# Complexity-ML/complexity-tokenizer

Measured on AMD Instinct MI355X. Metric: MB/s raw UTF-8 encoded (encode_batch), 50k ByteLevel BPE, 1/2/4/8 MI355X, higher is better.
Workload: dtype u8

## Files before the change

complexity-tokenizer_amd/csrc/ctok_internal.h:

```cpp
#pragma once
#include <hip/hip_runtime.h>

#include <cstdint>

namespace ctok_dev {

constexpr uint64_t kEmpty = ~0ull;
constexpr uint32_t kIdBits = 21;
constexpr uint64_t kKeyMask = (1ull << 42) - 1;
constexpr uint32_t kNoRank = 0x3FFFFFu;
constexpr uint32_t kMaxId = (1u << kIdBits) - 2;
constexpr uint32_t kPanicVal = kNoRank - 1;

constexpr uint32_t kErrPanic = 1u;

constexpr int kTileWords = 62;
constexpr int kTile = kTileWords * 64;
constexpr int kTileSlots = 4096;
constexpr int kSegWaves = 4;
constexpr int kSegUnroll = 4;
constexpr int kShortMax = 32;
constexpr int kMedMax = 64;
constexpr uint32_t kCap0 = kTile, kCap1 = (kTile + 8) / 9, kCap2 = (kTile + 16) / 17, kCap3 = (kTile + 32) / 33;
constexpr uint32_t kCap0Lean = 1040;
constexpr int kNumClasses = 4;
constexpr int kNumCounters = 32;
constexpr int kC3Shards = 64;
constexpr int kCounterWords = kNumCounters + kC3Shards;
__host__ __device__ constexpr int ctr_stat(int c) { return c < 3 ? 6 + 2 * c : 16; }
__host__ __device__ constexpr int ctr_chunk(int c) { return c < 3 ? 13 + c : 18; }
constexpr int kCtrLong = 0;
constexpr int kCtrErr = 2;
constexpr int kCtrNfcDocs = 3;
constexpr int kCtrDropped = 4;
constexpr int kCtrPieces = 5;
constexpr int kCtrNfcFlag = 12;
constexpr int kCtrAnyMid = 19;
constexpr int kCtrAnyC3 = 20;
constexpr int kCtrEmptyDocs = 21;
constexpr int kCtrC3Count = 22;
constexpr int kCtrC3Take = 23;
constexpr uint32_t kC3SparseDefault = 65536;
constexpr uint32_t kWgRecWords = 4 * 1024 * 4;
constexpr int kMidPackedDefault = 2;
constexpr int kOverlapDefault = 1;
constexpr int kCtrSink = 31;
constexpr int kCtrOverflow = 25;
constexpr int kCtrLongIds = 26;
constexpr int kCtrLwWords = 27;
constexpr int kCtrRounds = 29;
constexpr int kLhBuckets = 65;
constexpr int kLhHist = 0, kLhScan = 80, kLhFill = 160, kLhTake = 240, kLhWords = 320;
__host__ __device__ inline uint32_t long_bucket(uint32_t n) { return n > 4096 ? 0u : 64u - (n - 1) / 64; }
__host__ __device__ inline uint32_t list_entry(uint32_t sl, uint32_t o, uint32_t n) { return sl | (o << 12) | (n << 24); }
__host__ __device__ inline uint32_t ent_len(uint32_t e) { return (e >> 24) & 127u; }
__host__ __device__ inline uint32_t ent_ord(uint32_t e) { return (e >> 12) & 0xFFFu; }
__host__ __device__ inline uint32_t long_ord(uint64_t e) { return (uint32_t)(e >> 32) & 0xFFFu; }
__host__ __device__ inline uint32_t long_len(uint64_t e) { return (uint32_t)(e >> 44) & 0x7FFFFu; }

constexpr uint32_t kRecLong = 0x40000000u, kRecLongMask = kRecLong - 1u;
constexpr uint32_t kRecMerged32 = 0xFFFFFFFFu, kRecMerged16 = 0xFFFFu;
__host__ __device__ inline uint32_t region_base(uint2 r, int cls) {
  return cls <= 0 ? 0u : cls == 1 ? (r.x & 0xFFFFu) : cls == 2 ? (r.x >> 16) : r.y;
}
__host__ __device__ inline uint32_t rec_short(uint32_t count, uint32_t sl) { return count | (sl << 16); }

__host__ __device__ inline uint32_t mul24(uint32_t a, uint32_t b) {
#if defined(__HIP_DEVICE_COMPILE__)
  return __umul24(a, b);
#else
  return (a & 0xFFFFFFu) * (b & 0xFFFFFFu);
#endif
}

__host__ __device__ inline uint32_t mhash(uint32_t a, uint32_t b) {
  uint32_t h = mul24(a, 0x9E3779u) + mul24(b ^ 0x5A5A5Au, 0x85EBCBu);
  h ^= h >> 15;
  h = mul24(h, 0xC2B2AFu) ^ (h >> 9);
  return h ^ (h >> 16);
}
__host__ __device__ inline uint32_t mhash2(uint32_t h1) {
  uint32_t h = mul24(h1 ^ (h1 >> 24), 0x27D4EBu) + (h1 >> 11);
  h ^= h >> 13;
  h = mul24(h, 0x165667u) ^ (h >> 8);
  return h ^ (h >> 16);
}

constexpr uint32_t kHotBuckets = 4096;
constexpr uint32_t kBloomBits = 1u << 18;
constexpr uint32_t kHotU64 = 2 * kHotBuckets;
constexpr uint32_t kBloomWords = kBloomBits / 32;
constexpr uint32_t kLdsImageBytes = kHotU64 * 8 + kBloomWords * 4;
constexpr uint32_t kSortCap = 8192;

__host__ __device__ inline uint32_t key16(uint32_t a, uint32_t b) { return (a << 16) | b; }
__host__ __device__ inline uint32_t hash16_h(uint32_t a, uint32_t b) {
  const uint32_t h = mul24(a, 0x9E3779u) + mul24(b, 0x85EBCBu);
  return h ^ (h >> 13);
}
__host__ __device__ inline uint32_t hash16_g(uint32_t a, uint32_t b) {
  return mul24(b, 0xC2B2AFu) + mul24(a ^ 0x5A5Au, 0x27D4EBu);
}

__host__ __device__ inline uint32_t piece_hash(uint32_t lo, uint32_t hi, uint32_t len) {
  uint32_t h = mul24(lo, 0x9E3779u) + mul24((lo >> 24) | (hi << 8), 0x85EBCBu) + mul24((hi >> 16) | (len << 16), 0xC2B2AFu);
  h ^= h >> 15;
  h = mul24(h, 0x27D4EBu) ^ (h >> 9);
  return h ^ (h >> 16);
}

__host__ __device__ __forceinline__ int cp_range_class(uint32_t cp) {
  if (cp - 0x4E00u < 0x5200u) return 1;
  if (cp - 0xAC00u < 0x2BA4u) return 1;
  if (cp - 0x3041u < 0x56u) return 1;
  if (cp - 0x30A1u < 0x5Au) return 1;
  if (cp - 0x1F300u < 0x350u) return 3;
  return -1;
}

struct Tables {
  const uint64_t* merge_tab;
  uint32_t merge_mask;
  const uint4* lds_image;
  const uint32_t* pair0;
  const uint4* lds16_image;
  const uint64_t* merge16;
  uint32_t merge16_mask;
  const uint4* piece_tab;
  uint32_t piece_mask;
  const uint32_t* rank_newid;
  uint32_t n_ranks;
  const int32_t* byte2id;
  const uint8_t* cls_s1;
  const uint8_t* cls_s2;
  const uint8_t* nfc_s1;
  const uint16_t* nfc_s2;
  const uint8_t* cls_bmp;
  uint32_t cp_fast;
  const uint32_t* decomp_cp;
  const uint16_t* decomp_off;
  const uint32_t* decomp_data;
  uint32_t n_decomp;
  const uint64_t* comp_key;
  const uint32_t* comp_val;
  uint32_t n_comp;
  const uint8_t* bytemap_alnum;
  const uint8_t* at_bytes;
  const uint32_t* at_off;
  const uint32_t* at_id;
  const uint8_t* at_flags;
  uint32_t n_at;
  uint32_t proper;
  const uint32_t* eager;
  uint32_t window;
  const uint32_t* wmeta;
  uint32_t compact;
  uint32_t narrow;
  uint32_t short_packed;
  uint32_t mid_packed;
  uint32_t dbg;
  uint32_t all_bytes;
};

__host__ __device__ inline bool mid_folded(const Tables& t, uint32_t long_pieces) {
  return t.mid_packed == 2 && t.short_packed && t.n_at == 0 && long_pieces == 0;
}

struct Work {
  const uint8_t* text;
  uint32_t n_bytes;
  const uint64_t* doc_off;
  uint32_t n_docs;
  uint32_t* tfirst;
  uint32_t* pbits;
  uint32_t n_words;
  uint32_t n_tiles;
  uint32_t n_cus;
  uint32_t nfc_watch;
  uint32_t* nfc_bits;
  uint32_t mid_wide;
  uint32_t short_wgs;
  uint32_t chunk_sort;
  uint32_t keep_first;
  uint16_t* wpref;
  uint32_t* tile_np;
  uint32_t* tile_tok;
  uint32_t* tile_doc;
  uint32_t* tcls;
  uint32_t* list0;
  uint32_t k0;
  uint32_t* list1;
  uint32_t* list2;
  uint32_t* list3;
  void* prec;
  uint32_t rec16;
  uint32_t* mrec;
  uint32_t* pdoc;
  uint32_t* tcnt;
  uint32_t* long_cnt;
  uint32_t* long_ord;
  uint32_t* long_hist;
  uint32_t* scratch;
  uint32_t* lids;
  uint32_t* long_pos;
  uint32_t* lw_pos;
  uint32_t* rend;
  uint2* tregion;
  uint32_t long_cap, mid_cap;
  uint32_t unit;
  uint64_t* long_list;
  uint64_t* mid_list;
  uint32_t* counters;
  uint32_t* lw;
  uint32_t* scan_tmp;
  uint64_t scan_tmp_cap;
  uint64_t* stamps;
  uint32_t c3_max;
  uint32_t* c3q;
  uint32_t* c3pre;
  uint64_t* host_res;
  uint64_t* wgrec;
  uint32_t* report;
  uint32_t seq;
};

struct Lx {
  hipEvent_t start = nullptr, stop = nullptr;
};

constexpr uint32_t kDecLenMask = 0xFFFFFFu, kDecNonAscii = 1u << 30, kDecSpecial = 1u << 31;
constexpr uint32_t kDecOptSkipSpecial = 1u, kDecOptCleanup = 2u;
constexpr int kDecChunk = 4096;
constexpr int kDecTile = 4096;

struct DecTables {
  const uint2* ent;
  uint32_t n_ent;
  const uint8_t* bytes;
};

struct DecWork {
  const uint32_t* ids;
  uint32_t n_ids;
  const uint64_t* tok_off;
  uint32_t n_docs;
  uint32_t opts;
  uint32_t n_chunks;
  uint32_t* chunk_off;
  uint8_t* raw;
  uint32_t n_raw;
  uint64_t* raw_off;
  uint32_t* delbits;
  uint32_t n_tiles;
  uint32_t* tile_cnt;
  uint32_t* counters;
};

hipError_t launch_dec_len(const DecWork& w, const DecTables& t, uint32_t* tmp, uint64_t tmp_cap, hipStream_t s);
hipError_t launch_dec_gather(const DecWork& w, const DecTables& t, uint8_t* dst, uint64_t* dst_off, hipStream_t s);
hipError_t launch_dec_prepare(const DecWork& w, hipStream_t s);
hipError_t launch_dec_count(const DecWork& w, uint32_t* tmp, uint64_t tmp_cap, hipStream_t s);
hipError_t launch_dec_write(const DecWork& w, uint8_t* out, uint64_t* out_off, hipStream_t s);

constexpr uint32_t kPadItemA = 0xFFFFFFFFu;
constexpr int kPadMaxItems = 16;

struct PadWork {
  const uint32_t* ids;
  const uint64_t* tok_off;
  uint32_t n_rows;
  uint32_t pairs;
  uint32_t use_tpl;
  uint32_t n_items;
  uint32_t items[kPadMaxItems];
  uint32_t mark;
  const uint32_t* special_ids;
  uint32_t n_special;
  uint32_t truncate;
  uint64_t max_len;
  uint64_t target;
  uint32_t pad_left;
  uint32_t pad_id;
  uint64_t width;
  uint32_t* out_ids;
  uint32_t* out_attn;
  uint32_t* out_type;
  uint32_t* out_special;
  uint64_t* row_len;
  uint32_t* counters;
};
hipError_t launch_pad_len(const PadWork& w, hipStream_t s);
hipError_t launch_pad_rows(const PadWork& w, hipStream_t s);

struct WinWork {
  PadWork p;
  uint64_t stride;
  const uint32_t* tokenless;
  uint32_t n_tokenless;
  uint64_t ids_bound;
  uint64_t* row_win;
  uint64_t n_windows;
  uint64_t* win_len;
  uint32_t* win_row;
  uint64_t* win_start;
};
hipError_t launch_win_len(const WinWork& w, hipStream_t s);
hipError_t launch_win_rows(const WinWork& w, hipStream_t s);

void upload_done();
hipError_t launch_docstart(const Work& w, hipStream_t s, bool zero_counters, Lx x = {}, Lx x2 = {});
uint64_t nfc_bits_words(uint64_t n_bytes);
hipError_t scan_tiles(const Work& w, hipStream_t s, bool count, Lx x = {});
hipError_t launch_nfc_check(const uint8_t* text, uint64_t n_bytes, const uint64_t* doc_off, uint32_t n_docs,
                            const Tables& t, uint32_t* doc_flag, uint32_t* counter, hipStream_t s);
hipError_t launch_norm(const uint8_t* text, const uint64_t* doc_off, uint32_t n_docs, const uint32_t* doc_flag,
                       int add_prefix, int nfc, const Tables& t, uint32_t* cp_scratch, uint32_t* ncp,
                       uint64_t* new_len_then_off, uint8_t* out_text, int phase, hipStream_t s);
hipError_t launch_segment(const Work& w, const Tables& t, hipStream_t s, Lx x = {});
hipError_t launch_bpe_class(const Work& w, const Tables& t, int cls, hipStream_t s, Lx x = {});
hipError_t launch_report(const Work& w, hipStream_t s);
hipError_t launch_c3_sparse(const Work& w, const Tables& t, uint32_t n_pieces, hipStream_t s, Lx x = {});
hipError_t launch_long_prep(const Work& w, const Tables& t, hipStream_t s, uint32_t n_long, uint32_t* lwn,
                            uint32_t* tmp, uint64_t tmp_cap);
hipError_t launch_bpe_long(const Work& w, const Tables& t, hipStream_t s, uint32_t n_long, bool any_c3, bool any_gmem);
hipError_t launch_emit(const Work& w, uint32_t* ids, uint64_t ids_cap, uint64_t* tok_off, hipStream_t s,
                       bool count_pieces, bool empty_docs = true, Lx first = {}, Lx last = {});
hipError_t scan_u32(const uint32_t* in, uint32_t* out, uint64_t n_max, const uint32_t* n_dev,
                    uint32_t* tmp, uint64_t tmp_cap, hipStream_t s);
hipError_t scan_u64(uint64_t* inout, uint64_t n, uint64_t* tmp, uint64_t tmp_cap, hipStream_t s);
uint64_t scan_tmp_elems(uint64_t n_max);
uint64_t tile_scan_tmp_elems(uint64_t n_tiles);
hipError_t shift_u64(uint64_t* p, uint64_t n, uint64_t delta, hipStream_t s);
hipError_t launch_flag_docs(const uint64_t* off, uint64_t n_docs, const uint32_t* nfc_bits, uint32_t* flag, hipStream_t s);
hipError_t launch_flag_len(const uint64_t* off, const uint32_t* flag, uint64_t n_docs, uint64_t* len, hipStream_t s);
hipError_t launch_gather_flagged(const uint8_t* text, const uint64_t* off, const uint32_t* rank, const uint64_t* sub_pos,
                                 uint64_t n_docs, uint8_t* sub_text, uint64_t* sub_off, hipStream_t s);
hipError_t launch_splice(const uint32_t* rank, const uint64_t* main_off, const uint32_t* main_ids, const uint64_t* sub_off,
                         const uint32_t* sub_ids, uint64_t n_docs, uint32_t* ids, uint64_t ids_cap, uint64_t* out_off,
                         uint64_t* tmp, uint64_t tmp_cap, hipStream_t s);
hipError_t wire16(const uint32_t* ids, uint64_t n_ids, uint16_t* ids16, const uint64_t* toff, uint64_t n_off,
                  uint32_t* toff32, hipStream_t s);

}
```

complexity-tokenizer_amd/csrc/segment.hip:

```cpp
#include "dev_common.h"
#include "seg_lane.h"

namespace ctok_dev {


__global__ __launch_bounds__(256) void k_tilefirst(const uint64_t* __restrict__ off, uint32_t n_docs, uint32_t n_tiles,
                                                   uint32_t* __restrict__ tfirst, uint32_t* __restrict__ counters) {
  const uint32_t d = blockIdx.x * blockDim.x + threadIdx.x;
  bool empty = false;
  if (d <= n_docs && n_tiles) {
    const uint64_t y = off[d];
    empty = d < n_docs && y == off[d + 1];
    const uint64_t t_lo = d ? (off[d - 1] + 64) / kTile + 1 : 0ull;
    const uint64_t t_hi = min((y + 64) / kTile, (uint64_t)n_tiles - 1);
    for (uint64_t t = t_lo; t <= t_hi && t < t_lo + 64; t++) tfirst[t] = d;
  } else if (d < n_docs) {
    empty = off[d] == off[d + 1];
  }
  const uint64_t me = __ballot(empty);
  if (me && (threadIdx.x & 63) == (uint32_t)__ffsll((unsigned long long)me) - 1)
    atomicAdd(&counters[kCtrEmptyDocs], (uint32_t)__popcll(me));
}

__device__ uint32_t tile_first_search(const uint64_t* off, uint32_t n_docs, uint32_t tile) {
  const uint64_t key = tile ? (uint64_t)tile * kTile - 64 : 0ull;
  uint32_t lo = 0, hi = n_docs;
  while (lo < hi) {
    const uint32_t mid = lo + (hi - lo) / 2;
    if (__builtin_amdgcn_readfirstlane((uint32_t)(off[mid] < key))) lo = mid + 1;
    else hi = mid;
  }
  return lo;
}

__device__ __forceinline__ void clear_words(uint32_t* __restrict__ p, uint64_t n) {
  const uint64_t n4 = n / 4;
  uint4* p4 = reinterpret_cast<uint4*>(p);
  for (uint64_t i = (uint64_t)blockIdx.x * 256 + threadIdx.x; i < n4; i += (uint64_t)gridDim.x * 256)
    p4[i] = make_uint4(0u, 0u, 0u, 0u);
  if (blockIdx.x == 0 && threadIdx.x < n - 4 * n4) p[4 * n4 + threadIdx.x] = 0u;
}

__global__ __launch_bounds__(256) void k_clear(uint32_t* __restrict__ bits, uint64_t n, uint32_t* __restrict__ counters,
                                               uint32_t* __restrict__ tfirst, uint32_t n_tiles) {
  if (bits) clear_words(bits, n);
  for (uint32_t i = blockIdx.x * 256 + threadIdx.x; i < n_tiles; i += gridDim.x * 256) tfirst[i] = ~0u;
  if (blockIdx.x == 0 && counters && threadIdx.x < (uint32_t)kCounterWords) counters[threadIdx.x] = 0u;
}

uint64_t nfc_bits_words(uint64_t n_bytes) { return (n_bytes + 2047) / 2048 + 8; }

hipError_t launch_docstart(const Work& w, hipStream_t s, bool zero_counters, Lx x, Lx x2) {
  const bool nfc = w.nfc_watch == 2;
  const uint64_t n = nfc ? nfc_bits_words(w.n_bytes) : 0;
  const uint64_t work = std::max<uint64_t>(n / 4, w.n_tiles);
  launch_lx(x, k_clear, (unsigned)std::min<uint64_t>((work + 255) / 256 + 1, 8ull * w.n_cus), 256, 0, s,
            nfc ? w.nfc_bits : nullptr, n, zero_counters ? w.counters : nullptr, w.tfirst, w.n_tiles);
  if (w.n_tiles) launch_lx(x2, k_tilefirst, (w.n_docs + 1 + 255) / 256, 256, 0, s, w.doc_off, w.n_docs, w.n_tiles, w.tfirst, w.counters);
  else if (w.n_docs)
    k_tilefirst<<<(w.n_docs + 255) / 256, 256, 0, s>>>(w.doc_off, w.n_docs, 0, w.tfirst, w.counters);
  return hipGetLastError();
}


__device__ __forceinline__ uint32_t piece_probe(const Tables& t, uint4 e, uint32_t h, uint32_t lo, uint32_t hi,
                                                uint32_t n) {
  while (e.z != 0) {
    if (e.x == lo && e.y == hi && e.z == n) return e.w;
    h = (h + 1) & t.piece_mask;
    e = t.piece_tab[h];
  }
  return kNone;
}

__device__ __forceinline__ uint32_t select_bit(uint64_t x, uint32_t k) {
  uint32_t pos = 0;
  uint32_t lo = (uint32_t)x, hi = (uint32_t)(x >> 32);
  uint32_t c = __popc(lo);
  uint32_t v = lo;
  if (k >= c) { k -= c; v = hi; pos = 32; }
#pragma unroll
  for (int wdt = 16; wdt >= 1; wdt >>= 1) {
    const uint32_t m = (1u << wdt) - 1u;
    c = __popc(v & m);
    if (k >= c) { k -= c; v >>= wdt; pos += wdt; }
  }
  return pos;
}




#ifdef CTOK_SEG_STAMPS
#define SEG_STAMP(k)                                                                              \
  do {                                                                                            \
    __builtin_amdgcn_sched_barrier(0);                                                            \
    unsigned long long t_;                                                                        \
    asm volatile("s_memtime %0\n\ts_waitcnt lgkmcnt(0)" : "=s"(t_)::"memory");                     \
    __builtin_amdgcn_sched_barrier(0);                                                            \
    if (w.stamps && lane == 0) w.stamps[(size_t)tile * 8 + (k)] = t_;                            \
  } while (0)
#else
#define SEG_STAMP(k) do { } while (0)
#endif
template <bool R16>
__global__ __launch_bounds__(64 * kSegWaves) __attribute__((amdgpu_waves_per_eu(7))) void k_segment(Work w, Tables t) {
  __shared__ uint16_t s_pos_all[kSegWaves][64 * kSegUnroll + 8];
  __shared__ __attribute__((aligned(16))) uint32_t s_text_all[kSegWaves][(kTileWords + 2) * 16 + 8];
  __shared__ uint64_t s_D_all[kSegWaves][64];
  constexpr uint32_t kSegLongCap = 32;
  __shared__ uint64_t s_long_all[kSegWaves][kSegLongCap];
  const uint32_t lane = threadIdx.x & 63;
  const uint32_t wid = uni(threadIdx.x >> 6);
  const uint32_t tile = uni(blockIdx.x * kSegWaves + wid);
  if (tile >= w.n_tiles) return;
  uint16_t* s_pos = s_pos_all[wid];
  SEG_STAMP(0);
  const uint32_t B = w.n_bytes;
  const uint32_t t0 = tile * kTile;
  const int64_t g = (int64_t)tile * kTileWords - 1 + lane;
  const bool first = lane == 0, last = lane == 63;

  uint32_t x[16];
  uint64_t D, valid;
  {
    const int64_t x0 = g * 64;
    if (x0 >= 0 && x0 + 64 <= (int64_t)B) {
      const uint4* p = reinterpret_cast<const uint4*>(w.text + x0);
#pragma unroll
      for (int k = 0; k < 4; k++) {
        const uint4 v = p[k];
        x[4 * k] = v.x; x[4 * k + 1] = v.y; x[4 * k + 2] = v.z; x[4 * k + 3] = v.w;
      }
      valid = ~0ull;
    } else {
#pragma unroll
      for (int k = 0; k < 16; k++) x[k] = 0;
      valid = 0;
      if (x0 >= 0 && x0 < (int64_t)B) {
        const uint32_t n = B - (uint32_t)x0;
        valid = (1ull << n) - 1;
        for (uint32_t i = 0; i < n; i++) x[i >> 2] |= (uint32_t)w.text[x0 + i] << (8 * (i & 3));
      }
    }
  }
  uint32_t dfirst = uni(w.tfirst[tile]);
  if (dfirst == ~0u) dfirst = tile_first_search(w.doc_off, w.n_docs, tile);
  uint64_t xs0 = ~0ull, ys0 = ~0ull;
  if (dfirst + lane < w.n_docs) {
    xs0 = w.doc_off[dfirst + lane];
    ys0 = w.doc_off[dfirst + lane + 1];
  }
  seg::Masks m = seg::ascii_masks(x);
  {
    uint64_t* s_D = s_D_all[wid];
    s_D[lane] = 0;
    __builtin_amdgcn_fence(__ATOMIC_RELEASE, "wavefront");
    __builtin_amdgcn_wave_barrier();
    const uint64_t base = (uint64_t)t0 - 64;
    const uint64_t lim = (uint64_t)t0 + 4032;
    auto mark = [&](uint64_t xs, uint64_t ys) {
      const bool in = xs < lim;
      if (in && xs != ys) {
        const uint64_t r = xs - base;
        atomicOr((unsigned long long*)&s_D[r >> 6], 1ull << (r & 63));
      }
      return in;
    };
    if (__ballot(mark(xs0, ys0)) == ~0ull) {
      for (uint32_t d = dfirst + 64;; d += 64) {
        const uint32_t i = d + lane;
        uint64_t xs = ~0ull, ys = ~0ull;
        if (i < w.n_docs) {
          xs = w.doc_off[i];
          ys = w.doc_off[i + 1];
        }
        if (__ballot(mark(xs, ys)) != ~0ull) break;
      }
    }
    __builtin_amdgcn_fence(__ATOMIC_RELEASE, "wavefront");
    __builtin_amdgcn_wave_barrier();
    __builtin_amdgcn_fence(__ATOMIC_ACQUIRE, "wavefront");
    const int64_t x0 = g * 64;
    if (x0 < 0) D = 0;
    else if (x0 >= (int64_t)B) D = ~0ull;
    else D = s_D[lane] | ~valid;
  }
  s_D_all[wid][lane] = D;
  uint32_t* s_all = s_text_all[wid] + 4;
  uint32_t* s_text = s_all + 16;
  if (first && (x[0] & 0xC0u) == 0x80u && g * 64 >= 4)
    s_all[-1] = *reinterpret_cast<const uint32_t*>(w.text + g * 64 - 4);
#pragma unroll
  for (int k = 0; k < 4; k++)
    *reinterpret_cast<uint4*>(s_all + lane * 16 + 4 * k) = make_uint4(x[4 * k], x[4 * k + 1], x[4 * k + 2], x[4 * k + 3]);
  if (last) {
    const int64_t xe = g * 64 + 64;
    uint32_t v = 0;
    if (xe + 4 <= (int64_t)B) {
      v = *reinterpret_cast<const uint32_t*>(w.text + xe);
    } else {
      for (int64_t i = xe; i < (int64_t)B && i < xe + 4; i++) v |= (uint32_t)w.text[i] << (8 * (uint32_t)(i - xe));
    }
    s_all[64 * 16] = v;
  }
  __builtin_amdgcn_fence(__ATOMIC_RELEASE, "wavefront");
  __builtin_amdgcn_wave_barrier();
  __builtin_amdgcn_fence(__ATOMIC_ACQUIRE, "wavefront");
  SEG_STAMP(1);
  if (m.NA) {
    constexpr int kSegCp = 4;
    bool nfc_bad = false;
    auto set_class = [&](int cl, uint64_t bits) {
      if (cl == 0) m.W |= bits & m.NA;
      else if (cl == 1) m.L |= bits & m.NA;
      else if (cl == 2) m.N |= bits & m.NA;
    };
    uint64_t cont = 0;
#pragma unroll
    for (int k = 0; k < 16; k += 2) {
      const uint32_t c0 = x[k] & ~(x[k] << 1) & seg::kHi, c1 = x[k + 1] & ~(x[k + 1] << 1) & seg::kHi;
      cont |= (uint64_t)seg::pack8(c0, c1) << (4 * k);
    }
    cont &= m.NA;
    const uint64_t lead_cont = cont & ~(cont + 1);
    if (lead_cont) {
      const uint32_t pw = s_all[lane * 16 - 1];
      const int32_t back = ((pw >> 24) & 0xC0u) != 0x80u ? 1 : ((pw >> 16) & 0xC0u) != 0x80u ? 2 : 3;
      const int32_t a = (int32_t)lane * 64 - back;
      const uint32_t v = __builtin_amdgcn_alignbyte(s_all[(a >> 2) + 1], s_all[a >> 2], (uint32_t)a & 3u);
      const uint32_t b0 = v & 255u, b1 = (v >> 8) & 0x3Fu, b2 = (v >> 16) & 0x3Fu, b3 = (v >> 24) & 0x3Fu;
      const int l = u8len((uint8_t)b0);
      const uint32_t c = l == 2 ? ((b0 & 0x1Fu) << 6) | b1
                       : l == 3 ? ((b0 & 0x0Fu) << 12) | (b1 << 6) | b2
                       : l == 4 ? ((b0 & 0x07u) << 18) | (b1 << 12) | (b2 << 6) | b3 : b0;
      const int rc = t.cp_fast ? cp_range_class(c) : -1;
      const int cw = rc >= 0 ? rc : (cls_of(c, t) | (nfc16(t, c) != 0 ? 4 : 0));
      nfc_bad |= (cw & 4) != 0;
      set_class(cw & 3, lead_cont);
    }
    uint64_t leads = m.NA & ~cont;
    while (leads) {
      uint32_t pos[kSegCp], cp[kSegCp], len[kSegCp];
#pragma unroll
      for (int k = 0; k < kSegCp; k++) {
        pos[k] = leads ? (uint32_t)__builtin_ctzll(leads) : 64u;
        leads &= leads ? leads - 1 : 0ull;
      }
#pragma unroll
      for (int k = 0; k < kSegCp; k++) {
        const uint32_t a = lane * 64 + min(pos[k], 63u);
        const uint32_t v = __builtin_amdgcn_alignbyte(s_all[(a >> 2) + 1], s_all[a >> 2], a & 3);
        const uint32_t b0 = v & 255u, b1 = (v >> 8) & 0x3Fu, b2 = (v >> 16) & 0x3Fu, b3 = (v >> 24) & 0x3Fu;
        const int l = u8len((uint8_t)b0);
        len[k] = (uint32_t)l;
        cp[k] = l == 2 ? ((b0 & 0x1Fu) << 6) | b1
              : l == 3 ? ((b0 & 0x0Fu) << 12) | (b1 << 6) | b2
              : l == 4 ? ((b0 & 0x07u) << 18) | (b1 << 12) | (b2 << 6) | b3 : b0;
      }
      int rc[kSegCp];
      uint32_t s1[kSegCp];
#pragma unroll
      for (int k = 0; k < kSegCp; k++) {
        rc[k] = t.cp_fast ? cp_range_class(cp[k]) : -1;
        const bool in = pos[k] < 64 && cp[k] < 0x110000 && rc[k] < 0;
        s1[k] = in && cp[k] < 0x10000 ? (uint32_t)t.cls_bmp[cp[k] >> 1] : 0u;
      }
#pragma unroll
      for (int k = 0; k < kSegCp; k++) {
        if (pos[k] >= 64) continue;
        const uint32_t c = cp[k];
        int cl = 3;
        bool nf = false;
        if (rc[k] >= 0) {
          cl = rc[k];
        } else if (c < 0x80) {
          cl = cls_ascii(c);
        } else if (c < 0x10000) {
          const uint32_t v = s1[k] >> ((c & 1u) * 4);
          cl = (int)(v & 3u);
          nf = (v & 4u) != 0;
        } else if (c < 0x110000) {
          cl = cls_of(c, t);
          nf = nfc16(t, c) != 0;
        }
        nfc_bad |= nf;
        const uint32_t p = pos[k];
        const uint64_t bits = (len[k] >= 64 - p ? ~0ull : ((1ull << len[k]) - 1)) << p;
        set_class(cl, bits);
      }
    }
    if (nfc_bad && w.nfc_watch) {
      atomicOr(&w.counters[kCtrNfcFlag], 1u);
      if (w.nfc_watch == 2 && g >= 0) atomicOr(&w.nfc_bits[g >> 5], 1u << (g & 31));
    }
  }
  SEG_STAMP(2);
  uint64_t pQ = shfl_up64(m.Q);
  if (first) pQ = 0;
  seg::Letters lt{0, 0, 0, 0, 0};
  if (m.Q | (pQ >> 62)) lt = seg::letter_masks(x, m.NA);

  uint64_t st;
  {
    uint64_t pW = shfl_up64(m.W), pL = shfl_up64(m.L), pN = shfl_up64(m.N);
    if (first) pW = pL = pN = 0;
    uint64_t nW = shfl_down64(m.W), nL = shfl_down64(m.L), nD = shfl_down64(D);
    seg::Letters nl{shfl_down64(lt.T1), shfl_down64(lt.R), shfl_down64(lt.Le), shfl_down64(lt.V), shfl_down64(lt.LL)};
    if (last) {
      nW = nL = nD = 0;
      nl = seg::Letters{0, 0, 0, 0, 0};
    }
    const uint64_t A = seg::attached(m, D, pW, nW, nD);
    uint64_t pA = shfl_up64(A);
    if (first) pA = 0;
    uint64_t C1, C2;
    seg::contractions(m, lt, D, A, pA, ~(pW | pL | pN), nL, nD, nl, C1, C2);
    uint64_t pC1 = shfl_up64(C1), pC2 = shfl_up64(C2);
    if (first) pC1 = pC2 = 0;
    st = seg::starts(m, D, pW, pL, pN, A, pA, C1, C2, pC1, pC2) & valid;
    if (last) st &= (1ull << 62) - 1;
    if (!first && !last) {
      const uint64_t gw = (uint64_t)g * 2;
      if (gw < w.n_words) w.pbits[gw] = (uint32_t)st;
      if (gw + 1 < w.n_words) w.pbits[gw + 1] = (uint32_t)(st >> 32);
    }
  }
  uint32_t nd = (!first && !last) ? (uint32_t)__popcll(D & valid) : 0u;
  const uint32_t c = (!first && !last) ? (uint32_t)__popcll(st) : 0u;
  const uint32_t inc = wave_incl_scan(c);
  if (!first && !last) w.wpref[(size_t)tile * 64 + lane - 1] = (uint16_t)(inc - c);
  const uint32_t np = lane63(inc);
  const uint32_t tile_end =
      uni((uint32_t)__shfl((int)(st ? (uint32_t)(kTileWords * 64 + __builtin_ctzll(st))
                                    : ((uint64_t)B <= (uint64_t)t0 + kTile + 62 ? (uint32_t)(B - t0) : 0xFFFFu)),
                           63, 64));
  const uint64_t stw = (!first && !last) ? st : 0ull;
  const uint32_t prew = inc - c;
  uint32_t wcur = 1;

  SEG_STAMP(3);
  const bool generic = t.n_at != 0;
  using RecT = typename std::conditional<R16, uint16_t, uint32_t>::type;
  RecT* prec = (RecT*)w.prec + (size_t)tile * kTileSlots;
  uint32_t* pdoc = w.pdoc + (size_t)tile * (kTileSlots / 32);
  uint32_t hits = 0;
  uint32_t nm = 0;
  uint32_t n0 = 0, n1 = 0, n2 = 0, n3 = 0;
  uint32_t nlong = 0;
  uint32_t by0 = 0, by1 = 0, by2 = 0;
  constexpr int U = kSegUnroll;
  constexpr uint32_t W = 64 * U;
  for (uint32_t j0 = 0; j0 < np; j0 += W) {
    for (uint32_t wb = wcur;; wb += 32) {
      const uint32_t wl = wb + (lane >> 1), src = min(wl, 63u);
      const uint32_t lo32 = (uint32_t)__shfl((int)(uint32_t)stw, (int)src, 64);
      const uint32_t hi32 = (uint32_t)__shfl((int)(uint32_t)(stw >> 32), (int)src, 64);
      const uint32_t pw = (uint32_t)__shfl((int)prew, (int)src, 64);
      const bool hi = (lane & 1) != 0;
      uint32_t bits = wl <= (uint32_t)kTileWords ? (hi ? hi32 : lo32) : 0u;
      uint32_t k = pw + (hi ? (uint32_t)__popc(lo32) : 0u);
      if (k > j0 + W || k + (uint32_t)__popc(bits) <= j0) bits = 0;
      const uint32_t pos0 = (wl - 1) * 64 + (hi ? 32u : 0u);
      while (bits) {
        const uint32_t b = (uint32_t)__builtin_ctz(bits);
        if (k >= j0 && k <= j0 + W) s_pos[k - j0] = (uint16_t)(pos0 + b);
        bits &= bits - 1u;
        k++;
      }
      const uint32_t wn = wb + 32;
      if (wn > (uint32_t)kTileWords || uni(__builtin_amdgcn_readlane(prew, wn)) > j0 + W) break;
    }
    {
      const uint64_t inw = __ballot(lane >= wcur && lane <= (uint32_t)kTileWords && prew <= j0 + W);
      if (inw) wcur = 63u - (uint32_t)__builtin_clzll(inw);
    }

    if (lane == 0 && np <= j0 + W) s_pos[np - j0] = (uint16_t)tile_end;
    __builtin_amdgcn_fence(__ATOMIC_RELEASE, "wavefront");
    __builtin_amdgcn_wave_barrier();
    __builtin_amdgcn_fence(__ATOMIC_ACQUIRE, "wavefront");
    uint32_t sl[U], n[U], cls[U], plo[U], phi[U], h[U], doc[U];
#pragma unroll
    for (int u = 0; u < U; u++) {
      const uint32_t j = j0 + 64 * u + lane;
      sl[u] = 0;
      n[u] = 0;
      doc[u] = 0;
      cls[u] = 4;
      if (j < np) {
        sl[u] = s_pos[64 * u + lane];
        doc[u] = (uint32_t)(s_D_all[wid][(sl[u] >> 6) + 1] >> (sl[u] & 63)) & 1u;
        const uint32_t el = s_pos[64 * u + lane + 1];
        if (el == 0xFFFFu || el - sl[u] > (generic ? (uint32_t)kShortMax : (uint32_t)kMedMax)) {
          cls[u] = 3;
        } else {
          n[u] = el - sl[u];
          cls[u] = generic ? 0 : n[u] > 32 ? 6 : n[u] > 16 ? 2 : n[u] > 8 ? 1 : 5;
        }
      }
      const uint32_t a = sl[u] >> 2, sh = sl[u] & 3;
      const uint32_t d0 = s_text[a], d1 = s_text[a + 1], d2 = s_text[a + 2];
      const uint32_t w0 = __builtin_amdgcn_alignbyte(d1, d0, sh), w1 = __builtin_amdgcn_alignbyte(d2, d1, sh);
      const uint32_t nn = n[u];
      plo[u] = nn >= 4 ? w0 : w0 & ((1u << (8 * nn)) - 1u);
      phi[u] = nn >= 8 ? w1 : nn <= 4 ? 0u : w1 & ((1u << (8 * (nn - 4))) - 1u);
      h[u] = cls[u] == 5 ? piece_hash(plo[u], phi[u], nn) & t.piece_mask : t.piece_mask + 1;
    }
    uint32_t hitv[U];
#define CTOK_PROBE_LOAD(u) const uint4 e##u = t.piece_tab[h[u]];
#define CTOK_PROBE_USE(u) hitv[u] = piece_probe(t, e##u, h[u], plo[u], phi[u], n[u]);
    static_assert(U == 4 || U == 8, "kSegUnroll: 4 or 8");
    CTOK_PROBE_LOAD(0) CTOK_PROBE_LOAD(1) CTOK_PROBE_LOAD(2) CTOK_PROBE_LOAD(3)
    if constexpr (U == 8) {
      CTOK_PROBE_LOAD(4) CTOK_PROBE_LOAD(5) CTOK_PROBE_LOAD(6) CTOK_PROBE_LOAD(7)
      CTOK_PROBE_USE(4) CTOK_PROBE_USE(5) CTOK_PROBE_USE(6) CTOK_PROBE_USE(7)
    }
    CTOK_PROBE_USE(0) CTOK_PROBE_USE(1) CTOK_PROBE_USE(2) CTOK_PROBE_USE(3)
#undef CTOK_PROBE_LOAD
#undef CTOK_PROBE_USE
#pragma unroll
    for (int u = 0; u < U; u++) {
      const uint32_t j = j0 + 64 * u + lane;
      uint32_t rec = kRecMerged32;
      if (cls[u] == 5) {
        const bool hit = hitv[u] != kNone;
        rec = hit ? hitv[u] : kRecMerged32;
        hits += hit ? 1u : 0u;
        cls[u] = hit ? 4u : 0u;
      }
      if (j < np) {
        prec[j] = (RecT)rec;
      }
      const uint64_t dm = __ballot(j < np && doc[u]);
      if (lane == 0 && j0 + 64 * u < np)
        *reinterpret_cast<uint2*>(pdoc + ((j0 + 64 * u) >> 5)) = make_uint2((uint32_t)dm, (uint32_t)(dm >> 32));
    }
    {
      uint32_t tot0 = n0;
#pragma unroll
      for (int u = 0; u < U; u++) tot0 += (uint32_t)__popcll(__ballot(cls[u] == 0));
      if (tot0 > w.k0) {
        uint32_t c = n0;
#pragma unroll
        for (int u = 0; u < U; u++) {
          const uint64_t m = __ballot(cls[u] == 0);
          if (cls[u] == 0 && c + __popcll(m & lanemask_lt()) >= w.k0) cls[u] = 3;
          c += (uint32_t)__popcll(m);
        }
      }
    }
#pragma unroll
    for (int u = 0; u < U; u++) {
      const uint64_t below = lanemask_lt();
      const uint64_t mm = __ballot(cls[u] != 4);
      const uint32_t ord = nm + (uint32_t)__popcll(mm & below);
      nm += (uint32_t)__popcll(mm);
      const uint32_t e = list_entry(sl[u], ord, n[u]);
      {
        const uint64_t m0 = __ballot(cls[u] == 0);
        const uint64_t m1 = __ballot(cls[u] == 1), m2 = __ballot(cls[u] == 2);
        const uint64_t m3 = __ballot(cls[u] == 6);
        if (cls[u] == 0) w.list0[(size_t)tile * w.k0 + n0 + __popcll(m0 & below)] = e;
        if (cls[u] == 1) w.list1[(size_t)tile * kCap1 + n1 + __popcll(m1 & below)] = e;
        if (cls[u] == 2) w.list2[(size_t)tile * kCap2 + n2 + __popcll(m2 & below)] = e;
        if (cls[u] == 6) w.list3[(size_t)tile * kCap3 + n3 + __popcll(m3 & below)] = e;
        by0 += cls[u] == 0 ? n[u] : 0u;
        by1 += cls[u] == 1 ? n[u] : 0u;
        by2 += cls[u] == 2 ? n[u] : 0u;
        n0 += __popcll(m0);
        n1 += __popcll(m1);
        n2 += __popcll(m2);
        n3 += __popcll(m3);
      }
      const uint64_t lm = __ballot(cls[u] == 3);
      if (lm && nlong + (uint32_t)__popcll(lm) <= kSegLongCap) {
        if (cls[u] == 3) {
          const uint32_t el = s_pos[64 * u + lane + 1];
          const uint32_t ln = el == 0xFFFFu ? 0u : min(el - sl[u], 0x7FFFFu);
          s_long_all[wid][nlong + __popcll(lm & lanemask_lt())] =
              (uint64_t)(t0 + sl[u]) | ((uint64_t)ord << 32) | ((uint64_t)ln << 44);
        }
        nlong += (uint32_t)__popcll(lm);
      } else if (lm) {
        const uint32_t leader = __ffsll((unsigned long long)lm) - 1;
        uint32_t b = 0;
        if (lane == leader) b = atomicAdd(&w.counters[kCtrLong], (uint32_t)__popcll(lm));
        b = __builtin_amdgcn_readlane(b, leader);
        const uint32_t li = b + __popcll(lm & lanemask_lt());
        if (cls[u] == 3 && li < w.long_cap)
        {
          const uint32_t el = s_pos[64 * u + lane + 1];
          const uint32_t ln = el == 0xFFFFu ? 0u : min(el - sl[u], 0x7FFFFu);
          w.long_list[li] = (uint64_t)(t0 + sl[u]) | ((uint64_t)ord << 32) | ((uint64_t)ln << 44);
        }
        if (lane == leader && b + __popcll(lm) > w.long_cap) atomicOr(&w.counters[kCtrOverflow], 1u);
      }
    }
    __builtin_amdgcn_fence(__ATOMIC_RELEASE, "wavefront");
    __builtin_amdgcn_wave_barrier();
    __builtin_amdgcn_fence(__ATOMIC_ACQUIRE, "wavefront");
  }
  if (nlong) {
    uint32_t b = 0;
    if (lane == 0) b = atomicAdd(&w.counters[kCtrLong], nlong);
    b = __builtin_amdgcn_readfirstlane(b);
    __builtin_amdgcn_fence(__ATOMIC_RELEASE, "wavefront");
    __builtin_amdgcn_wave_barrier();
    __builtin_amdgcn_fence(__ATOMIC_ACQUIRE, "wavefront");
    if (lane < nlong && b + lane < w.long_cap) w.long_list[b + lane] = s_long_all[wid][lane];
    if (lane == 0 && b + nlong > w.long_cap) atomicOr(&w.counters[kCtrOverflow], 1u);
  }
  SEG_STAMP(4);
  hits = wave_sum_full_u32(hits);
  by0 = wave_sum_full_u32(by0);
  by1 = wave_sum_full_u32(by1);
  by2 = wave_sum_full_u32(by2);
  nd = wave_sum_full_u32(nd);
  if (lane == 0) {
    w.tile_tok[tile] = hits;
    w.tile_doc[tile] = nd;
    w.tile_np[tile] = np;
    w.tregion[tile] = make_uint2(by0 | ((by0 + by1) << 16), by0 + by1 + by2);
  }
  if (lane < kNumClasses)
    w.rend[(size_t)lane * w.n_tiles + tile] = lane == 0 ? 0u : lane == 1 ? by0 : lane == 2 ? by0 + by1 : by0 + by1 + by2;
  if (lane < kNumClasses)
    w.tcls[(size_t)lane * w.n_tiles + tile] = lane == 0 ? n0 : lane == 1 ? n1 : lane == 2 ? n2 : n3;
  if (lane == 0 && n2) w.counters[kCtrAnyMid] = 1;
  if (lane == 0 && n3) w.counters[kCtrAnyC3] = 1;
  if (n3 && w.c3_max) {
    const uint32_t sh = tile & (kC3Shards - 1), cap = w.c3_max / kC3Shards;
    uint32_t b = 0;
    if (lane == 0) b = atomicAdd(&w.counters[kNumCounters + sh], n3);
    b = __builtin_amdgcn_readfirstlane(b);
    for (uint32_t j = lane; j < n3; j += 64)
      if (b + j < cap) w.c3q[(size_t)sh * cap + b + j] = (tile << 7) | j;
  }
  SEG_STAMP(5);
#ifdef CTOK_SEG_STAMPS
  if (w.stamps && lane == 0) w.stamps[(size_t)tile * 8 + 6] = np;
#endif
}

hipError_t launch_segment(const Work& w, const Tables& t, hipStream_t s, Lx x) {
  const uint32_t grid = (w.n_tiles + kSegWaves - 1) / kSegWaves;
  if (w.n_tiles && w.rec16) launch_lx(x, k_segment<true>, grid, 64 * kSegWaves, 0, s, w, t);
  else if (w.n_tiles) launch_lx(x, k_segment<false>, grid, 64 * kSegWaves, 0, s, w, t);
  return hipGetLastError();
}

}
```

Before: 176,500.

## Compact non-hit pieces into LDS buffer before emitting class lists

```diff
diff --git a/complexity-tokenizer_amd/csrc/ctok_internal.h b/complexity-tokenizer_amd/csrc/ctok_internal.h
--- a/complexity-tokenizer_amd/csrc/ctok_internal.h
+++ b/complexity-tokenizer_amd/csrc/ctok_internal.h
@@ -19,6 +19,10 @@
 constexpr int kTileSlots = 4096;
 constexpr int kSegWaves = 4;
 constexpr int kSegUnroll = 4;
+constexpr uint32_t kSegListBuf = 64 * kSegUnroll;
+__host__ __device__ inline uint32_t seg_mark(uint32_t sl, uint32_t cls) { return sl | (cls << 12); }
+__host__ __device__ inline uint32_t seg_mark_start(uint32_t m) { return m & 0xFFFu; }
+__host__ __device__ inline uint32_t seg_mark_class(uint32_t m) { return m >> 12; }
 constexpr int kShortMax = 32;
 constexpr int kMedMax = 64;
 constexpr uint32_t kCap0 = kTile, kCap1 = (kTile + 8) / 9, kCap2 = (kTile + 16) / 17, kCap3 = (kTile + 32) / 33;
diff --git a/complexity-tokenizer_amd/csrc/segment.hip b/complexity-tokenizer_amd/csrc/segment.hip
--- a/complexity-tokenizer_amd/csrc/segment.hip
+++ b/complexity-tokenizer_amd/csrc/segment.hip
@@ -71,6 +71,12 @@
     e = t.piece_tab[h];
   }
   return kNone;
+}
+
+__device__ __forceinline__ void seg_wave_sync() {
+  __builtin_amdgcn_fence(__ATOMIC_RELEASE, "wavefront");
+  __builtin_amdgcn_wave_barrier();
+  __builtin_amdgcn_fence(__ATOMIC_ACQUIRE, "wavefront");
 }
 
 __device__ __forceinline__ uint32_t select_bit(uint64_t x, uint32_t k) {
@@ -110,6 +116,7 @@
   __shared__ uint64_t s_D_all[kSegWaves][64];
   constexpr uint32_t kSegLongCap = 32;
   __shared__ uint64_t s_long_all[kSegWaves][kSegLongCap];
+  __shared__ uint8_t s_buf_all[kSegWaves][kSegListBuf];
   const uint32_t lane = threadIdx.x & 63;
   const uint32_t wid = uni(threadIdx.x >> 6);
   const uint32_t tile = uni(blockIdx.x * kSegWaves + wid);
@@ -178,9 +185,7 @@
         if (__ballot(mark(xs, ys)) != ~0ull) break;
       }
     }
-    __builtin_amdgcn_fence(__ATOMIC_RELEASE, "wavefront");
-    __builtin_amdgcn_wave_barrier();
-    __builtin_amdgcn_fence(__ATOMIC_ACQUIRE, "wavefront");
+    seg_wave_sync();
     const int64_t x0 = g * 64;
     if (x0 < 0) D = 0;
     else if (x0 >= (int64_t)B) D = ~0ull;
@@ -204,9 +209,7 @@
     }
     s_all[64 * 16] = v;
   }
-  __builtin_amdgcn_fence(__ATOMIC_RELEASE, "wavefront");
-  __builtin_amdgcn_wave_barrier();
-  __builtin_amdgcn_fence(__ATOMIC_ACQUIRE, "wavefront");
+  seg_wave_sync();
   SEG_STAMP(1);
   if (m.NA) {
     constexpr int kSegCp = 4;
@@ -326,7 +329,7 @@
       if (gw + 1 < w.n_words) w.pbits[gw + 1] = (uint32_t)(st >> 32);
     }
   }
-  uint32_t nd = (!first && !last) ? (uint32_t)__popcll(D & valid) : 0u;
+  const uint32_t nd = uni(wave_sum_full_u32((!first && !last) ? (uint32_t)__popcll(D & valid) : 0u));
   const uint32_t c = (!first && !last) ? (uint32_t)__popcll(st) : 0u;
   const uint32_t inc = wave_incl_scan(c);
   if (!first && !last) w.wpref[(size_t)tile * 64 + lane - 1] = (uint16_t)(inc - c);
@@ -344,13 +347,67 @@
   using RecT = typename std::conditional<R16, uint16_t, uint32_t>::type;
   RecT* prec = (RecT*)w.prec + (size_t)tile * kTileSlots;
   uint32_t* pdoc = w.pdoc + (size_t)tile * (kTileSlots / 32);
-  uint32_t hits = 0;
   uint32_t nm = 0;
   uint32_t n0 = 0, n1 = 0, n2 = 0, n3 = 0;
   uint32_t nlong = 0;
-  uint32_t by0 = 0, by1 = 0, by2 = 0;
+  uint32_t by01 = 0, by2h = 0;
   constexpr int U = kSegUnroll;
   constexpr uint32_t W = 64 * U;
+  static_assert(U == 4, "kSegUnroll: 4 (the probes of a round are unrolled by hand)");
+  static_assert(kSegListBuf == W && W <= 256, "s_buf: a whole round's pieces, one byte each");
+  uint8_t* s_buf = s_buf_all[wid];
+  uint32_t cnt = 0;
+  auto flush = [&]() __attribute__((always_inline)) {
+    const uint64_t below = lanemask_lt();
+    for (uint32_t p0 = 0; p0 < cnt; p0 += 64) {
+      const uint32_t i = p0 + lane, ord = nm + i;
+      uint32_t bsl = 0, bn = 0;
+      uint32_t cl = 4;
+      if (i < cnt) {
+        const uint32_t k = s_buf[i];
+        const uint32_t a = s_pos[k], el = s_pos[k + 1];
+        bsl = seg_mark_start(a);
+        cl = seg_mark_class(a);
+        bn = el == 0xFFFFu ? 0u : seg_mark_start(el) - bsl;
+      }
+      uint64_t m0 = __ballot(cl == 0);
+      if (n0 + (uint32_t)__popcll(m0) > w.k0) {
+        if (cl == 0 && n0 + (uint32_t)__popcll(m0 & below) >= w.k0) cl = 3;
+        m0 = __ballot(cl == 0);
+      }
+      const uint32_t e = list_entry(bsl, ord, bn);
+      {
+        const uint64_t m1 = __ballot(cl == 1), m2 = __ballot(cl == 2);
+        const uint64_t m3 = __ballot(cl == 6);
+        if (cl == 0) w.list0[(size_t)tile * w.k0 + n0 + __popcll(m0 & below)] = e;
+        if (cl == 1) w.list1[(size_t)tile * kCap1 + n1 + __popcll(m1 & below)] = e;
+        if (cl == 2) w.list2[(size_t)tile * kCap2 + n2 + __popcll(m2 & below)] = e;
+        if (cl == 6) w.list3[(size_t)tile * kCap3 + n3 + __popcll(m3 & below)] = e;
+        by01 += cl == 0 ? bn : cl == 1 ? bn << 16 : 0u;
+        by2h += cl == 2 ? bn : 0u;
+        n0 += __popcll(m0);
+        n1 += __popcll(m1);
+        n2 += __popcll(m2);
+        n3 += __popcll(m3);
+      }
+      const uint64_t lm = __ballot(cl == 3);
+      const uint64_t le = (uint64_t)(t0 + bsl) | ((uint64_t)ord << 32) | ((uint64_t)bn << 44);
+      if (lm && nlong + (uint32_t)__popcll(lm) <= kSegLongCap) {
+        if (cl == 3) s_long_all[wid][nlong + __popcll(lm & below)] = le;
+        nlong += (uint32_t)__popcll(lm);
+      } else if (lm) {
+        const uint32_t leader = __ffsll((unsigned long long)lm) - 1;
+        uint32_t b = 0;
+        if (lane == leader) b = atomicAdd(&w.counters[kCtrLong], (uint32_t)__popcll(lm));
+        b = __builtin_amdgcn_readlane(b, leader);
+        const uint32_t li = b + __popcll(lm & below);
+        if (cl == 3 && li < w.long_cap) w.long_list[li] = le;
+        if (lane == leader && b + __popcll(lm) > w.long_cap) atomicOr(&w.counters[kCtrOverflow], 1u);
+      }
+    }
+    nm += cnt;
+    cnt = 0;
+  };
   for (uint32_t j0 = 0; j0 < np; j0 += W) {
     for (uint32_t wb = wcur;; wb += 32) {
       const uint32_t wl = wb + (lane >> 1), src = min(wl, 63u);
@@ -377,9 +434,7 @@
     }
 
     if (lane == 0 && np <= j0 + W) s_pos[np - j0] = (uint16_t)tile_end;
-    __builtin_amdgcn_fence(__ATOMIC_RELEASE, "wavefront");
-    __builtin_amdgcn_wave_barrier();
-    __builtin_amdgcn_fence(__ATOMIC_ACQUIRE, "wavefront");
+    seg_wave_sync();
     uint32_t sl[U], n[U], cls[U], plo[U], phi[U], h[U], doc[U];
 #pragma unroll
     for (int u = 0; u < U; u++) {
@@ -410,12 +465,7 @@
     uint32_t hitv[U];
 #define CTOK_PROBE_LOAD(u) const uint4 e##u = t.piece_tab[h[u]];
 #define CTOK_PROBE_USE(u) hitv[u] = piece_probe(t, e##u, h[u], plo[u], phi[u], n[u]);
-    static_assert(U == 4 || U == 8, "kSegUnroll: 4 or 8");
     CTOK_PROBE_LOAD(0) CTOK_PROBE_LOAD(1) CTOK_PROBE_LOAD(2) CTOK_PROBE_LOAD(3)
-    if constexpr (U == 8) {
-      CTOK_PROBE_LOAD(4) CTOK_PROBE_LOAD(5) CTOK_PROBE_LOAD(6) CTOK_PROBE_LOAD(7)
-      CTOK_PROBE_USE(4) CTOK_PROBE_USE(5) CTOK_PROBE_USE(6) CTOK_PROBE_USE(7)
-    }
     CTOK_PROBE_USE(0) CTOK_PROBE_USE(1) CTOK_PROBE_USE(2) CTOK_PROBE_USE(3)
 #undef CTOK_PROBE_LOAD
 #undef CTOK_PROBE_USE
@@ -426,97 +476,42 @@
       if (cls[u] == 5) {
         const bool hit = hitv[u] != kNone;
         rec = hit ? hitv[u] : kRecMerged32;
-        hits += hit ? 1u : 0u;
+        by2h += hit ? 0x10000u : 0u;
         cls[u] = hit ? 4u : 0u;
       }
       if (j < np) {
         prec[j] = (RecT)rec;
       }
-      const uint64_t dm = __ballot(j < np && doc[u]);
+      const uint64_t dm = __ballot(doc[u] != 0);
       if (lane == 0 && j0 + 64 * u < np)
         *reinterpret_cast<uint2*>(pdoc + ((j0 + 64 * u) >> 5)) = make_uint2((uint32_t)dm, (uint32_t)(dm >> 32));
     }
-    {
-      uint32_t tot0 = n0;
-#pragma unroll
-      for (int u = 0; u < U; u++) tot0 += (uint32_t)__popcll(__ballot(cls[u] == 0));
-      if (tot0 > w.k0) {
-        uint32_t c = n0;
-#pragma unroll
-        for (int u = 0; u < U; u++) {
-          const uint64_t m = __ballot(cls[u] == 0);
-          if (cls[u] == 0 && c + __popcll(m & lanemask_lt()) >= w.k0) cls[u] = 3;
-          c += (uint32_t)__popcll(m);
-        }
-      }
-    }
+    seg_wave_sync();
 #pragma unroll
     for (int u = 0; u < U; u++) {
-      const uint64_t below = lanemask_lt();
       const uint64_t mm = __ballot(cls[u] != 4);
-      const uint32_t ord = nm + (uint32_t)__popcll(mm & below);
-      nm += (uint32_t)__popcll(mm);
-      const uint32_t e = list_entry(sl[u], ord, n[u]);
-      {
-        const uint64_t m0 = __ballot(cls[u] == 0);
-        const uint64_t m1 = __ballot(cls[u] == 1), m2 = __ballot(cls[u] == 2);
-        const uint64_t m3 = __ballot(cls[u] == 6);
-        if (cls[u] == 0) w.list0[(size_t)tile * w.k0 + n0 + __popcll(m0 & below)] = e;
-        if (cls[u] == 1) w.list1[(size_t)tile * kCap1 + n1 + __popcll(m1 & below)] = e;
-        if (cls[u] == 2) w.list2[(size_t)tile * kCap2 + n2 + __popcll(m2 & below)] = e;
-        if (cls[u] == 6) w.list3[(size_t)tile * kCap3 + n3 + __popcll(m3 & below)] = e;
-        by0 += cls[u] == 0 ? n[u] : 0u;
-        by1 += cls[u] == 1 ? n[u] : 0u;
-        by2 += cls[u] == 2 ? n[u] : 0u;
-        n0 += __popcll(m0);
-        n1 += __popcll(m1);
-        n2 += __popcll(m2);
-        n3 += __popcll(m3);
-      }
-      const uint64_t lm = __ballot(cls[u] == 3);
-      if (lm && nlong + (uint32_t)__popcll(lm) <= kSegLongCap) {
-        if (cls[u] == 3) {
-          const uint32_t el = s_pos[64 * u + lane + 1];
-          const uint32_t ln = el == 0xFFFFu ? 0u : min(el - sl[u], 0x7FFFFu);
-          s_long_all[wid][nlong + __popcll(lm & lanemask_lt())] =
-              (uint64_t)(t0 + sl[u]) | ((uint64_t)ord << 32) | ((uint64_t)ln << 44);
-        }
-        nlong += (uint32_t)__popcll(lm);
-      } else if (lm) {
-        const uint32_t leader = __ffsll((unsigned long long)lm) - 1;
-        uint32_t b = 0;
-        if (lane == leader) b = atomicAdd(&w.counters[kCtrLong], (uint32_t)__popcll(lm));
-        b = __builtin_amdgcn_readlane(b, leader);
-        const uint32_t li = b + __popcll(lm & lanemask_lt());
-        if (cls[u] == 3 && li < w.long_cap)
-        {
-          const uint32_t el = s_pos[64 * u + lane + 1];
-          const uint32_t ln = el == 0xFFFFu ? 0u : min(el - sl[u], 0x7FFFFu);
-          w.long_list[li] = (uint64_t)(t0 + sl[u]) | ((uint64_t)ord << 32) | ((uint64_t)ln << 44);
-        }
-        if (lane == leader && b + __popcll(lm) > w.long_cap) atomicOr(&w.counters[kCtrOverflow], 1u);
-      }
-    }
-    __builtin_amdgcn_fence(__ATOMIC_RELEASE, "wavefront");
-    __builtin_amdgcn_wave_barrier();
-    __builtin_amdgcn_fence(__ATOMIC_ACQUIRE, "wavefront");
+      if (cls[u] != 4) {
+        s_pos[64 * u + lane] = (uint16_t)seg_mark(sl[u], cls[u]);
+        s_buf[cnt + (uint32_t)__popcll(mm & lanemask_lt())] = (uint8_t)(64 * u + lane);
+      }
+      cnt += (uint32_t)__popcll(mm);
+    }
+    seg_wave_sync();
+    flush();
+    seg_wave_sync();
   }
   if (nlong) {
     uint32_t b = 0;
     if (lane == 0) b = atomicAdd(&w.counters[kCtrLong], nlong);
     b = __builtin_amdgcn_readfirstlane(b);
-    __builtin_amdgcn_fence(__ATOMIC_RELEASE, "wavefront");
-    __builtin_amdgcn_wave_barrier();
-    __builtin_amdgcn_fence(__ATOMIC_ACQUIRE, "wavefront");
+    seg_wave_sync();
     if (lane < nlong && b + lane < w.long_cap) w.long_list[b + lane] = s_long_all[wid][lane];
     if (lane == 0 && b + nlong > w.long_cap) atomicOr(&w.counters[kCtrOverflow], 1u);
   }
   SEG_STAMP(4);
-  hits = wave_sum_full_u32(hits);
-  by0 = wave_sum_full_u32(by0);
-  by1 = wave_sum_full_u32(by1);
-  by2 = wave_sum_full_u32(by2);
-  nd = wave_sum_full_u32(nd);
+  by01 = wave_sum_full_u32(by01);
+  by2h = wave_sum_full_u32(by2h);
+  const uint32_t by0 = by01 & 0xFFFFu, by1 = by01 >> 16, by2 = by2h & 0xFFFFu, hits = by2h >> 16;
   if (lane == 0) {
     w.tile_tok[tile] = hits;
     w.tile_doc[tile] = nd;
```

Result: faster. 179,600, median of 6 (+1.8%).
